# tangtang888/video-edge-ai-proxy

Hardware: AMD Instinct MI355X
Metric: decoded FPS (whole node) + p50 VideoLatestImage latency, 256×1080p RTSP (higher is better)
Workload: dtype uint8 (BGR24 frames; bf16-capable consumer path)

## Files before the change

csrc/vep/gpu_avc.hip:

```cpp
#define VEP_KERNEL_SOURCE 1
#include "avc_recon.h"
#include "gpu.h"

namespace vep::gpu {

using avc::MbRec;
using avc::kDenseCoefs;

namespace {

constexpr int kIntraWaves = kAvcDbkWgRows;
constexpr int kIntraXgWords = 8;
constexpr int kIntraLine = 32;
constexpr int kIntraLineCols = 240;
constexpr u32 kSpinLimit = 1u << 24;

__device__ inline const MbRec& rec(const AvcDesc& d, int mb) {
  return static_cast<const MbRec*>(d.mbs)[mb];
}


__device__ inline void wave_sync() {
  __builtin_amdgcn_fence(__ATOMIC_RELEASE, "wavefront");
  __builtin_amdgcn_wave_barrier();
// ... 435 lines not shown
        avc::intra16x16_const_from_sums(m.i16_mode, B, A, st, sl, H, V, P(15, -1), P(-1, 15));
    auto T = [&](int xx) { return P(xx, -1); };
    auto Lf = [&](int yy) { return P(-1, yy); };
    u8 out[4];
    for (int k = 0; k < 4; ++k) {
      const int p = lane + 64 * k, px = p & 15, py = p >> 4;
      out[k] = u8(avc::clip1(avc::intra16x16_pred_g(T, Lf, pk, m.i16_mode, px, py) + L.res[p]));
    }
    wave_sync();
    for (int k = 0; k < 4; ++k) {
      const int p = lane + 64 * k;
      L.tile[((p >> 4) + 1) * kTp + (p & 15) + 1] = out[k];
    }
  } else if (m.kind == avc::kI8x8) {
    const int px = lane & 7, py = lane >> 3;
    for (int q = 0; q < 4; ++q) {
      const int bx = q & 1, by = q >> 1;
      const bool top = by > 0 || B, left = bx > 0 || A;
      const bool tl = (bx > 0 && by > 0) || (bx == 0 && by == 0 ? D : bx == 0 ? A : B);
      const bool tr = by == 0 ? (bx == 0 ? B : C) : (bx == 0);
      const u8* nb = &L.tile[(by * 8) * kTp + bx * 8];
      const int mode = avc::i4_mode(m, q);
      const int rs = L.res[(by * 8 + py) * 16 + bx * 8 + px];
      const u32 pw = tap8_lut[mode * 64 + lane];
      if (lane < 25) {
        const u32 fw = avc::intra8x8_filter_tap(top, left, tl, lane);
        auto off = [&](u32 u) -> int { return u > 16 ? int(u - 16) * kTp : (u >= 9 && !tr) ? 8 : int(u); };
        const int s0 = nb[off(fw & 31)], s1 = nb[off((fw >> 5) & 31)], s2 = nb[off((fw >> 10) & 31)];
        const int fv = avc::eval_tap8(fw, s0, s1, s2);
        L.pf[lane] = u8((fw & avc::kTap8Const) ? 128 : fv);
      }
      wave_sync();
      int v;
      if (mode == 2) {
        int sv = lane < 8 ? (top ? int(L.pf[1 + lane]) : 0) : lane < 16 ? (left ? int(L.pf[9 + lane]) : 0) : 0;
        for (int o = 8; o > 0; o >>= 1) sv += __shfl_xor(sv, o);
        sv = __shfl(sv, 0);
        v = top && left ? (sv + 8) >> 4 : (top || left) ? (sv + 4) >> 3 : 128;
      } else {
        v = avc::eval_tap8(pw, L.pf[pw & 31], L.pf[(pw >> 5) & 31], L.pf[(pw >> 10) & 31]);
      }
      L.tile[(by * 8 + py + 1) * kTp + bx * 8 + px + 1] = u8(avc::clip1(v + rs));
      wave_sync();
    }
  } else {
    for (int k = 0; k < 4; ++k) {
      const int p = lane + 64 * k, px = p & 15, py = p >> 4, bx = px >> 2, byy = py >> 2;
      const int r = byy * 4 + bx;
      const u32 tw = tap_lut[avc::i4_mode(m, r) * 16 + (py & 3) * 4 + (px & 3)];
      u32 word;
      if (tw & avc::kTapDc) {
        word = 1u << 31 | u32(byy > 0 || B) << 21 | u32(bx > 0 || A) << 22;
      } else {
        const bool tr = byy == 0 ? (bx < 3 ? B : C)
                                 : (bx < 3 && avc::raster_to_blk((byy - 1) * 4 + bx + 1) < avc::raster_to_blk(r));
        auto rel = [&](u32 n) -> u32 {
          return n == 0 ? 0u : n <= 8 ? 1u + ((n - 1 >= 4 && !tr) ? 3u : n - 1) : (n - 8) * u32(kTp);
        };
        word = rel(tw & 15) | rel((tw >> 4) & 15) << 7 | rel((tw >> 8) & 15) << 14 | ((tw >> 12) & 1023u) << 21;
      }
      L.taps[p] = word;
    }
    wave_sync();
    const int g = lane >> 4, i = (lane >> 2) & 3, j = lane & 3;
    auto slot = [&](int st) -> int {
      const int y_lo = st > 3 ? (st - 2) / 2 : 0, y_hi = st / 2 < 3 ? st / 2 : 3;
      const int yy = y_lo + g;
      return g < 2 && yy <= y_hi ? (yy * 4 + i) * 16 + (st - 2 * yy) * 4 + j : -1;
    };
    u32 tws[10];
    int rss[10];
#pragma unroll
    for (int st = 0; st < 10; ++st) {
      const int p = slot(st);
      tws[st] = p >= 0 ? L.taps[p] : 0u;
      rss[st] = p >= 0 ? L.res[p] : 0;
    }
#pragma unroll
    for (int st = 0; st < 10; ++st) {
      const int p = slot(st);
      if (p >= 0) {
        const int yy = p >> 6, bx = (p & 15) >> 2;
        const u32 tw = tws[st];
        const u8* nb = &L.tile[(yy * 4) * kTp + bx * 4];
        int v;
        if (tw >> 31) {
          int st4 = 0, sl4 = 0;
          for (int q = 0; q < 4; ++q) {
            st4 += nb[1 + q];
            sl4 += nb[(q + 1) * kTp];
          }
          const bool ht = (tw >> 21) & 1, hl = (tw >> 22) & 1;
          v = ht && hl ? (st4 + sl4 + 4) >> 3 : hl ? (sl4 + 2) >> 2 : ht ? (st4 + 2) >> 2 : 128;
        } else {
          const int n0 = nb[tw & 127], n1 = nb[(tw >> 7) & 127], n2 = nb[(tw >> 14) & 127];
          v = (int((tw >> 21) & 3) * n0 + int((tw >> 23) & 3) * n1 + int((tw >> 25) & 3) * n2 +
               int((tw >> 27) & 3)) >> int((tw >> 29) & 3);
        }
        v += rss[st];
        L.tile[(yy * 4 + i + 1) * kTp + bx * 4 + j + 1] = u8(avc::clip1(v));
      }
      wave_sync();
    }
  }
  const u64 t_luma = d.prof ? clock64() : 0;
  {
    u8 out[2];
    for (int k = 0; k < 2; ++k) {
      const int p = lane + 64 * k, c = p >> 6, q = p & 63, px = q & 7, py = q >> 3;
      const u8* t = L.ctile[c];
      auto T = [&](int xx) { return int(t[xx + 1]); };
      auto Lf = [&](int yy) { return int(t[(yy + 1) * kCp]); };
      const avc::PredConst pk =
          m.chroma_mode == 3 ? avc::chroma_plane_const_g(T, Lf) : avc::PredConst{0, 0, 0, 0};
      out[k] = u8(avc::clip1(avc::chroma_pred_g(T, Lf, B, A, pk, m.chroma_mode, px, py) + L.res[256 + p]));
    }
    wave_sync();
    for (int k = 0; k < 2; ++k) {
      const int p = lane + 64 * k, c = p >> 6, q = p & 63;
      L.ctile[c][((q >> 3) + 1) * kCp + (q & 7) + 1] = out[k];
    }
  }
  wave_sync();
  const u64 t_chroma = d.prof ? clock64() : 0;
  {
    const int ry = lane >> 2, rx = (lane & 3) * 4;
    const u8* src = &L.tile[(ry + 1) * kTp + rx + 1];
    const u32 w = u32(src[0]) | u32(src[1]) << 8 | u32(src[2]) << 16 | u32(src[3]) << 24;
    gst4(Y + size_t(y0 + ry) * pitch + x0 + rx, w);
    if (xi_out && lane >= 60) xg_put(xi_out + size_t(x) * kAvcXgWords + (lane - 60), w, 1u);
    if (line_out && lane >= 60) *(VEP_LDS u32*)(line_out + x * kIntraLine + (lane - 60) * 4) = w;
    if (lane < 32) {
      const int cyr = lane >> 2, cxb = (lane & 3) * 2;
      const u8* c0 = &L.ctile[0][(cyr + 1) * kCp + cxb + 1];
      const u8* c1 = &L.ctile[1][(cyr + 1) * kCp + cxb + 1];
      const u32 cw = u32(c0[0]) | u32(c1[0]) << 8 | u32(c0[1]) << 16 | u32(c1[1]) << 24;
      gst4(UV + size_t(row * 8 + cyr) * pitch + (x * 8 + cxb) * 2, cw);
      if (xi_out && lane >= 28) xg_put(xi_out + size_t(x) * kAvcXgWords + 4 + (lane - 28), cw, 1u);
      if (line_out && lane >= 28) *(VEP_LDS u32*)(line_out + x * kIntraLine + 16 + (lane - 28) * 4) = cw;
    }
    if (lane < 16) L.carry[lane] = L.tile[(lane + 1) * kTp + 16];
    if (lane < 16) L.ccarry[lane >> 3][lane & 7] = L.ctile[lane >> 3][((lane & 7) + 1) * kCp + 8];
  }
  wave_sync();
  if (d.prof) {
    __builtin_amdgcn_fence(__ATOMIC_RELEASE, "workgroup");
    const u64 t_end = clock64();
    acc[1] += t_loaded - t_start - waited;
    acc[2] += t_luma - t_res;
    acc[6] += t_res - t_loaded;
    acc[3] += t_chroma - t_luma;
    acc[4] += t_end - t_chroma;
    acc[5] += 1;
  }
}

__global__ __launch_bounds__(64 * kIntraWaves) void avc_intra_kernel(const AvcDesc* __restrict__ descs,
                                                                      int n, int groups) {
  const int b = int(blockIdx.x), j = b >> 3;
  const int pic = (j / groups) * 8 + (b & 7), grp = j % groups;
  if (pic >= n) return;
  const AvcDesc d = descs[pic];
  const int W = d.wmbs, H = d.hmbs, g0 = grp * kIntraWaves;
  if (g0 >= H || d.bd > 8 || d.cf == 2) return;
  __shared__ Sync sync;
  __shared__ IntraWave lds[kIntraWaves];
  __shared__ u32 tap_lut[9 * 16];
  __shared__ u32 tap8_lut[9 * 64];
  __shared__ u8 lines[kIntraWaves - 1][kIntraLineCols * kIntraLine];
  for (int t = int(threadIdx.x); t < 9 * 16; t += int(blockDim.x)) {
    const int mode = t >> 4, y = (t >> 2) & 3, x = t & 3;
    tap_lut[t] = mode == 2 ? avc::kTapDc : avc::pack_taps(avc::intra4x4_taps(mode, x, y));
  }
  for (int t = int(threadIdx.x); t < 9 * 64; t += int(blockDim.x))
    tap8_lut[t] = avc::intra8x8_pred_tap(t >> 6, t & 7, (t >> 3) & 7);
  sync_init(sync, kIntraWaves);
  const int wave = int(threadIdx.x) >> 6, lane = int(threadIdx.x) & 63;
  IntraWave& L = lds[wave];
  const MbRec* recs = static_cast<const MbRec*>(d.mbs);
  const int row = g0 + wave;
  const bool xin = grp > 0 && wave == 0;
  u64* xi_in = xin ? d.xg + size_t(grp - 1) * W * kAvcXgWords : nullptr;
  u64* xi_out = wave == kIntraWaves - 1 && row + 1 < H ? d.xg + size_t(grp) * W * kAvcXgWords : nullptr;
  const bool use_lines = W <= kIntraLineCols;
  const u8* line_in = use_lines && wave > 0 ? lines[wave - 1] : nullptr;
  u8* line_out = use_lines && wave + 1 < kIntraWaves ? lines[wave] : nullptr;
  u64 acc[7] = {0, 0, 0, 0, 0, 0, 0};
  if (row < H) {
    int prev = -2;
    for (int base = 0; base < W; base += 64) {
      const int x = base + lane;
      bool intra = false;
      if (x < W) {
        constexpr int kWords = int(sizeof(MbRec) / sizeof(uint2));
        const uint2* src = reinterpret_cast<const uint2*>(&recs[row * W + x]);
        uint2* dst = reinterpret_cast<uint2*>(&L.rec[lane]);
        uint2 q[kWords];
        for (int k = 0; k < kWords; ++k) q[k] = gld8(src + k);
        for (int k = 0; k < kWords; ++k) dst[k] = q[k];
        intra = avc::is_wave_intra(u8(q[0].x & 0xff));
      }
      if (row > 0)
        for (int q = lane; q < 66; q += 64) {
          const int ax = base - 1 + q;
          u8 v = 0;
          if (ax >= 0 && ax < W) {
            v = avc::is_wave_intra(u8(gld1(&recs[(row - 1) * W + ax].kind)));
          }
          L.up[q] = v;
        }
      const u64 mask = __ballot(intra);
      wave_sync();
      for (u64 bits = mask; bits; bits &= bits - 1) {
        const int xx = base + __ffsll(static_cast<unsigned long long>(bits)) - 1;
        const u64 t0 = d.prof ? clock64() : 0;
        publish_row(sync, wave, u32(xx));
        intra_mb(d, L, L.rec[xx - base], xx, row, prev == xx - 1, lane, tap_lut, tap8_lut, t0, acc, sync, wave,
                 wave > 0 ? u32(xx + 2 < W ? xx + 2 : W) : 0u, xi_in, row > 0 ? &L.up[1] - base : nullptr,
                 line_in, line_out, xi_out);
        prev = xx;
      }
    }
    publish_row(sync, wave, u32(W));
  }
  if (d.prof && lane == 0) {
    for (int k = 0; k < 6; ++k) atomicAdd(&d.prof[k], acc[k]);
    atomicAdd(&d.prof[11], acc[6]);
  }
}


__global__ __launch_bounds__(256) void avc_bs_kernel(const AvcDesc* __restrict__ descs, int n,
                                                      int total) {
  const int g = int(blockIdx.x) * 256 + int(threadIdx.x);
  if (g >= total) return;
  int lo = 0, hi = n - 1;
  while (lo < hi) {
    const int mid = (lo + hi + 1) >> 1;
    if (descs[mid].mb_begin <= g) lo = mid;
    else hi = mid - 1;
  }
  const AvcDesc d = descs[lo];
  const int mb = g - d.mb_begin, W = d.wmbs, x = mb % W, row = mb / W;
  if (row % kAvcDbkWgRows == kAvcDbkWgRows - 1 && row + 1 < d.hmbs) {
    uint4* z = reinterpret_cast<uint4*>(
        d.xg + (size_t(row / kAvcDbkWgRows) * W + x) * kAvcXgWords);
    for (int k = 0; k < kAvcXgWords / 2; ++k) z[k] = make_uint4(0, 0, 0, 0);
  }
  const MbRec q = rec(d, mb);
  AvcDbkInfo info{};
  if (!(q.dbk & 1)) {
    const MbRec lm = rec(d, x > 0 ? mb - 1 : mb);
    const MbRec tm = rec(d, row > 0 ? mb - W : mb);
    const bool left = x > 0 && !((q.dbk & 2) && lm.slice != q.slice);
    const bool top = row > 0 && !((q.dbk & 2) && tm.slice != q.slice);
    const i16* mq = avc::is_intra(q.kind) ? nullptr : d.mvs + size_t(q.mv);
    const i16* ml = avc::is_intra(lm.kind) ? nullptr : d.mvs + size_t(lm.mv);
    const i16* mt = avc::is_intra(tm.kind) ? nullptr : d.mvs + size_t(tm.mv);
    const bool t8 = (q.flags & avc::kMbT8x8) != 0;
    const avc::BsSide sq = avc::bs_side(q), sl = avc::bs_side(lm), st = avc::bs_side(tm);
    u64 bsw[2] = {0, 0};
    for (int dir = 0; dir < 2; ++dir)
      for (int e = 0; e < 4; ++e) {
        if (e == 0 && !(dir == 0 ? left : top)) continue;
        if ((e & 1) && t8 && !(d.cf == 2 && dir == 1)) continue;
        const avc::BsSide p = e > 0 ? sq : (dir == 0 ? sl : st);
        const i16* mp = e > 0 ? mq : (dir == 0 ? ml : mt);
        for (int sg = 0; sg < 4; ++sg) {
          const int bq = dir == 0 ? sg * 4 + e : e * 4 + sg;
          const int bp = e > 0 ? (dir == 0 ? bq - 1 : bq - 4) : (dir == 0 ? bq + 3 : bq + 12);
          const int bs = avc::boundary_strength(p, bp, mp, sq, bq, mq, e == 0, d.field != 0, dir == 0);
          const u64 v = u64(bs) << (4 * (e * 4 + sg));
          if (dir == 0) bsw[0] |= v;
          else bsw[1] |= v;
        }
      }
    info.bs[0] = u32(bsw[0]);
    info.bs[1] = u32(bsw[0] >> 32);
    info.bs[2] = u32(bsw[1]);
    info.bs[3] = u32(bsw[1] >> 32);
    info.any = (bsw[0] | bsw[1]) ? 1 : 0;
    const int qb = d.qp_bias, qcb = d.qpc_bias;
#pragma unroll
    for (int k = 0; k < 3; ++k) {
      const MbRec& pk = k == 0 ? lm : (k == 1 ? tm : q);
      const avc::EdgeParams ep[3] = {avc::edge_params(pk.qp - qb, q.qp - qb, q.alpha_off, q.beta_off),
                                     avc::edge_params(pk.qpc - qcb, q.qpc - qcb, q.alpha_off, q.beta_off),
                                     avc::edge_params(pk.qpc2 - qcb, q.qpc2 - qcb, q.alpha_off, q.beta_off)};
      for (int c = 0; c < 3; ++c) {
        info.alpha[c * 3 + k] = u8(ep[c].alpha);
        info.beta[c * 3 + k] = u8(ep[c].beta);
        for (int j = 0; j < 3; ++j) info.tc0[c * 3 + k][j] = u8(ep[c].tc0[j]);
      }
    }
  }
  static_cast<AvcDbkInfo*>(d.dbk)[mb] = info;
}


struct DbkWave {
  AvcDbkInfo info;
  u8 y[20 * 20];
  u8 c[2][10 * 12];
  u8 carry[16 * 4];
  u8 ccarry[2][8 * 2];
};

struct alignas(16) DbkXch {
  u8 y[4 * 16];
  u8 c[2 * 16];
};

constexpr int kDbkLag = 1;
constexpr int kDbkDepth = 8;
#ifndef VEP_DBK_WG_ROWS
#define VEP_DBK_WG_ROWS kAvcDbkWgRows
#endif
constexpr int kDbkRows = VEP_DBK_WG_ROWS;
constexpr int kDbkWaves = kDbkRows / 2;
constexpr u32 kXgFinal = 2u, kXgPartial = 1u;
static_assert(kDbkRows % 2 == 0 && kDbkDepth > kDbkLag && kDbkRows % kAvcDbkWgRows == 0 && kDbkRows <= 32,
              "deblock wavefront geometry");

struct DbkSync {
  u32 progress[kDbkRows];
  u32 abort;
};

__device__ inline void st4(u8* p, u32 v) { *reinterpret_cast<u32*>(p) = v; }
__device__ inline u32 ld4(const u8* p) { return *reinterpret_cast<const u32*>(p); }

__device__ inline void wait_row_lds(DbkSync& s, int r, u32 need, u32* err) {
  u32 spins = 0;
  while (__hip_atomic_load(&s.progress[r], __ATOMIC_RELAXED, __HIP_MEMORY_SCOPE_WORKGROUP) < need) {
    if (__hip_atomic_load(&s.abort, __ATOMIC_RELAXED, __HIP_MEMORY_SCOPE_WORKGROUP)) break;
    if (++spins > kSpinLimit) {
      __hip_atomic_store(&s.abort, 1u, __ATOMIC_RELAXED, __HIP_MEMORY_SCOPE_WORKGROUP);
      if ((threadIdx.x & 63) == 0) atomicOr(err, 2u);
      break;
    }
    __builtin_amdgcn_s_sleep(1);
  }
  __builtin_amdgcn_fence(__ATOMIC_ACQUIRE, "workgroup", "local");
}

__device__ inline int bs_of(const AvcDbkInfo& in, int dir, int e, int sg) {
  const int i = dir * 16 + e * 4 + sg;
  return int((in.bs[i >> 3] >> (4 * (i & 7))) & 15u);
}

__device__ inline bool filter_vals(int p0, int p1, int p2, int p3, int q0, int q1, int q2, int q3, int bs, int alpha,
                                   int beta, int tc0, bool chroma, int& np0, int& np1, int& np2, int& nq0, int& nq1,
                                   int& nq2) {
  if (!(avc::iabs(p0 - q0) < alpha && avc::iabs(p1 - p0) < beta && avc::iabs(q1 - q0) < beta)) return false;
  const int ap = avc::iabs(p2 - p0), aq = avc::iabs(q2 - q0);
  const bool lp = !chroma && ap < beta, lq = !chroma && aq < beta;
  np1 = p1;
  nq1 = q1;
  np2 = p2;
  nq2 = q2;
  if (bs < 4) {
    const int tc = chroma ? tc0 + 1 : tc0 + int(lp) + int(lq);
    const int dl = avc::clip3(-tc, tc, (((q0 - p0) << 2) + (p1 - q1) + 4) >> 3);
    np0 = avc::clip1(p0 + dl);
    nq0 = avc::clip1(q0 - dl);
    if (lp) np1 = p1 + avc::clip3(-tc0, tc0, (p2 + ((p0 + q0 + 1) >> 1) - (p1 << 1)) >> 1);
    if (lq) nq1 = q1 + avc::clip3(-tc0, tc0, (q2 + ((p0 + q0 + 1) >> 1) - (q1 << 1)) >> 1);
  } else {
    const bool strong = !chroma && avc::iabs(p0 - q0) < ((alpha >> 2) + 2);
    if (lp && strong) {
      np0 = (p2 + 2 * p1 + 2 * p0 + 2 * q0 + q1 + 4) >> 3;
      np1 = (p2 + p1 + p0 + q0 + 2) >> 2;
      np2 = (2 * p3 + 3 * p2 + p1 + p0 + q0 + 4) >> 3;
    } else {
      np0 = (2 * p1 + p0 + q1 + 2) >> 2;
    }
    if (lq && strong) {
      nq0 = (p1 + 2 * p0 + 2 * q0 + 2 * q1 + q2 + 4) >> 3;
      nq1 = (p0 + q0 + q1 + q2 + 2) >> 2;
      nq2 = (2 * q3 + 3 * q2 + q1 + q0 + p0 + 4) >> 3;
    } else {
      nq0 = (2 * q1 + q0 + p1 + 2) >> 2;
    }
  }
  return true;
}

__device__ inline void filter_vert_any(u8* q0p, int bs, int alpha, int beta, int tc0, bool chroma) {
  int p0, p1, p2, p3, q0, q1, q2, q3;
  u32 P = 0, Q = 0;
  if (!chroma) {
    const u32* w = reinterpret_cast<const u32*>(q0p - 4);
    P = w[0];
    Q = w[1];
    p3 = int(P & 255);
    p2 = int((P >> 8) & 255);
    p1 = int((P >> 16) & 255);
    p0 = int(P >> 24);
    q0 = int(Q & 255);
    q1 = int((Q >> 8) & 255);
    q2 = int((Q >> 16) & 255);
    q3 = int(Q >> 24);
  } else {
    const u16* h = reinterpret_cast<const u16*>(q0p - 2);
    P = h[0];
    Q = h[1];
    p1 = p2 = p3 = int(P & 255);
    p0 = int(P >> 8);
    q0 = int(Q & 255);
    q1 = q2 = q3 = int(Q >> 8);
  }
  int np0, np1, np2, nq0, nq1, nq2;
  if (!filter_vals(p0, p1, p2, p3, q0, q1, q2, q3, bs, alpha, beta, tc0, chroma, np0, np1, np2, nq0, nq1, nq2)) return;
  if (!chroma) {
    u32* w = reinterpret_cast<u32*>(q0p - 4);
    w[0] = (P & 255u) | u32(np2) << 8 | u32(np1) << 16 | u32(np0) << 24;
    w[1] = u32(nq0) | u32(nq1) << 8 | u32(nq2) << 16 | (Q & 0xFF000000u);
  } else {
    u16* h = reinterpret_cast<u16*>(q0p - 2);
    h[0] = u16((P & 255u) | u32(np0) << 8);
    h[1] = u16(u32(nq0) | (Q & 0xFF00u));
  }
}

__device__ inline void filter_line_any(u8* s, int step, int bs, int alpha, int beta, int tc0, bool chroma) {
  const int p0 = s[-step], p1 = s[-2 * step], q0 = s[0], q1 = s[step];
  const int p2 = s[-3 * step], p3 = s[-4 * step], q2 = s[2 * step], q3 = s[3 * step];
  if (!(avc::iabs(p0 - q0) < alpha && avc::iabs(p1 - p0) < beta && avc::iabs(q1 - q0) < beta)) return;
  const int ap = avc::iabs(p2 - p0), aq = avc::iabs(q2 - q0);
  const bool lp = !chroma && ap < beta, lq = !chroma && aq < beta;
  int np0, nq0, np1 = p1, nq1 = q1, np2 = p2, nq2 = q2;
  if (bs < 4) {
    const int tc = chroma ? tc0 + 1 : tc0 + int(lp) + int(lq);
    const int dl = avc::clip3(-tc, tc, (((q0 - p0) << 2) + (p1 - q1) + 4) >> 3);
    np0 = avc::clip1(p0 + dl);
    nq0 = avc::clip1(q0 - dl);
    if (lp) np1 = p1 + avc::clip3(-tc0, tc0, (p2 + ((p0 + q0 + 1) >> 1) - (p1 << 1)) >> 1);
    if (lq) nq1 = q1 + avc::clip3(-tc0, tc0, (q2 + ((p0 + q0 + 1) >> 1) - (q1 << 1)) >> 1);
  } else {
    const bool strong = !chroma && avc::iabs(p0 - q0) < ((alpha >> 2) + 2);
    if (lp && strong) {
      np0 = (p2 + 2 * p1 + 2 * p0 + 2 * q0 + q1 + 4) >> 3;
      np1 = (p2 + p1 + p0 + q0 + 2) >> 2;
      np2 = (2 * p3 + 3 * p2 + p1 + p0 + q0 + 4) >> 3;
    } else {
      np0 = (2 * p1 + p0 + q1 + 2) >> 2;
    }
    if (lq && strong) {
      nq0 = (p1 + 2 * p0 + 2 * q0 + 2 * q1 + q2 + 4) >> 3;
      nq1 = (p0 + q0 + q1 + q2 + 2) >> 2;
      nq2 = (2 * q3 + 3 * q2 + q1 + q0 + p0 + 4) >> 3;
    } else {
      nq0 = (2 * q1 + q0 + p1 + 2) >> 2;
    }
  }
  s[-step] = u8(np0);
  s[0] = u8(nq0);
  if (!chroma) {
    s[-2 * step] = u8(np1);
    s[step] = u8(nq1);
    s[-3 * step] = u8(np2);
    s[2 * step] = u8(nq2);
  }
}

__device__ inline void dbk_dir(DbkWave& L, bool any, int l, int dir, bool packed, bool sync_each) {
  const bool ch = l >= 16;
  const int c = (l - 16) >> 3, k = (l - 16) & 7;
  int bs[4], al[4], be[4], tc[4];
#pragma unroll
  for (int e = 0; e < 4; ++e) {
    bs[e] = any && (!ch || !(e & 1)) ? bs_of(L.info, dir, e, ch ? k >> 1 : l >> 2) : 0;
    const int pi = (e > 0 ? 2 : dir) + (ch ? 3 + 3 * c : 0);
    al[e] = L.info.alpha[pi];
    be[e] = L.info.beta[pi];
    tc[e] = L.info.tc0[pi][bs[e] > 0 && bs[e] < 4 ? bs[e] - 1 : 0];
  }
#pragma unroll
  for (int e = 0; e < 4; ++e) {
    if (bs[e] && dir == 0 && packed) {
      u8* q0p = !ch ? &L.y[(4 + l) * 20 + 4 + 4 * e] : &L.c[c][(2 + k) * 12 + 4 + 2 * e];
      filter_vert_any(q0p, bs[e], al[e], be[e], bs[e] < 4 ? tc[e] : 0, ch);
    } else if (bs[e]) {
      u8* sp;
      int step;
      if (!ch) {
        sp = dir == 0 ? &L.y[(4 + l) * 20 + 4 + 4 * e] : &L.y[(4 + 4 * e) * 20 + 4 + l];
        step = dir == 0 ? 1 : 20;
      } else {
        sp = dir == 0 ? &L.c[c][(2 + k) * 12 + 4 + 2 * e] : &L.c[c][(2 + 2 * e) * 12 + 4 + k];
        step = dir == 0 ? 1 : 12;
      }
      filter_line_any(sp, step, bs[e], al[e], be[e], bs[e] < 4 ? tc[e] : 0, ch);
    }
    if (sync_each) wave_sync();
  }
  if (!sync_each) wave_sync();
}

__device__ inline void dbk_dir_regs(DbkWave& L, bool any, int l, int dir) {
  const bool ch = l >= 16;
  const int c = (l - 16) >> 3, k = (l - 16) & 7;
  int bs[4], al[4], be[4], tc[4];
#pragma unroll
  for (int e = 0; e < 4; ++e) {
    const int ee = ch ? 2 * e : e;
    bs[e] = any && (!ch || e < 2) ? bs_of(L.info, dir, ee, ch ? k >> 1 : l >> 2) : 0;
    const int pi = (ee > 0 ? 2 : dir) + (ch ? 3 + 3 * c : 0);
    al[e] = L.info.alpha[pi];
    be[e] = L.info.beta[pi];
    tc[e] = L.info.tc0[pi][bs[e] > 0 && bs[e] < 4 ? bs[e] - 1 : 0];
  }
  u32 w[5] = {0, 0, 0, 0, 0};
  u8* row = !ch ? &L.y[(4 + l) * 20] : &L.c[c][(2 + k) * 12];
  u8* col = !ch ? &L.y[4 * 20 + 4 + l] : &L.c[c][2 * 12 + 4 + k];
  const int stride = ch ? 12 : 20, lo = ch ? 2 : 0, hi = ch ? 12 : 20, nw = ch ? 3 : 5;
  if (dir == 0) {
#pragma unroll
    for (int i = 0; i < 5; ++i)
      if (i < nw) w[i] = ld4(row + 4 * i);
  } else {
#pragma unroll
    for (int i = 0; i < 20; ++i)
      if (i >= lo && i < hi) w[i >> 2] |= u32(col[(i - 4) * stride]) << (8 * (i & 3));
  }
#pragma unroll
  for (int e = 0; e < 4; ++e) {
    if (!bs[e]) continue;
    const u32 P = w[e], Q = w[e + 1];
    int np0, np1, np2, nq0, nq1, nq2;
    if (!filter_vals(int(P >> 24), int((P >> 16) & 255), int((P >> 8) & 255), int(P & 255), int(Q & 255),
                     int((Q >> 8) & 255), int((Q >> 16) & 255), int(Q >> 24), bs[e], al[e], be[e],
                     bs[e] < 4 ? tc[e] : 0, ch, np0, np1, np2, nq0, nq1, nq2))
      continue;
    w[e] = (P & 255u) | u32(np2) << 8 | u32(np1) << 16 | u32(np0) << 24;
    w[e + 1] = u32(nq0) | u32(nq1) << 8 | u32(nq2) << 16 | (Q & 0xFF000000u);
  }
  if (dir == 0) {
#pragma unroll
    for (int i = 0; i < 5; ++i)
      if (i < nw) st4(row + 4 * i, w[i]);
  } else {
#pragma unroll
    for (int i = 1; i < 20; ++i)
      if (i >= lo && i < hi) col[(i - 4) * stride] = u8(w[i >> 2] >> (8 * (i & 3)));
  }
  wave_sync();
}

struct DbkRegs {
  u32 info, m0, m1, c;
};

__global__ __launch_bounds__(64 * kDbkWaves) void avc_deblock_kernel(const AvcDesc* __restrict__ descs,
                                                                      int n, int groups, int packed) {
  const int b = int(blockIdx.x), j = b >> 3;
  const int pic = (j / groups) * 8 + (b & 7), grp = j % groups;
  if (pic >= n) return;
  const AvcDesc d = descs[pic];
  const int W = d.wmbs, H = d.hmbs, pitch = W * 16;
  const int g0 = grp * kDbkRows;
  if (g0 >= H || d.bd > 8 || d.cf == 2) return;
  __shared__ DbkSync sync;
  __shared__ DbkWave lds[kDbkWaves][2];
  __shared__ DbkXch xring[kDbkRows - 1][kDbkDepth];
  if (threadIdx.x < kDbkRows) sync.progress[threadIdx.x] = 0;
  if (threadIdx.x == 0) sync.abort = 0;
  __syncthreads();
  const int wave = int(threadIdx.x) >> 6, lane = int(threadIdx.x) & 63;
  const int h = lane >> 5, l = lane & 31;
  DbkWave& L = lds[wave][h];
  u8* Y = d.y + d.slot_y * u64(d.target);
  u8* UV = d.uv + d.slot_uv * u64(d.target);
  const AvcDbkInfo* infos = static_cast<const AvcDbkInfo*>(d.dbk);
  auto xch = [&](int r, int x) -> DbkXch& { return xring[r - g0][x % kDbkDepth]; };
  auto load_mb = [&](int row, int x) {
    row = row < H ? row : H - 1;
    x = x < 0 ? 0 : (x < W ? x : W - 1);
    DbkRegs v;
    v.info = gld4(reinterpret_cast<const u32*>(&infos[size_t(row) * W + x]) + (l < 16 ? l : 0));
    const u8* ym = Y + size_t(row * 16 + (l >> 2)) * pitch + x * 16 + (l & 3) * 4;
    v.m0 = gld4(ym);
    v.m1 = gld4(ym + size_t(8) * pitch);
    v.c = gld4(UV + size_t(row * 8 + (l >> 2)) * pitch + x * 16 + (l & 3) * 4);
    return v;
  };
  const int r0 = g0 + 2 * wave, row = r0 + h, lrow = row - g0;
  const bool last = row == H - 1;
  const bool prod = row + 1 < H;
  const bool xout = prod && lrow == kDbkRows - 1;
  const bool xin = grp > 0 && wave == 0;
  const int xw = l >= 16 ? l - 16 : (l >= 8 ? 16 + (l - 8) : -1);
  const bool xneed = xin && h == 0 && xw >= 0;
  u64* xg_in = xin ? d.xg + size_t(grp - 1) * W * kAvcXgWords : nullptr;
  u64* xg_out = d.xg + size_t(grp) * W * kAvcXgWords;
  u64 gx = 0;
  if (xneed) gx = xg_get(xg_in + xw);
  u64 acc[5] = {0, 0, 0, 0, 0};
  DbkRegs cur = load_mb(row, -kDbkLag * h);
  for (int i = 0; r0 < H && i < W + kDbkLag; ++i) {
    const int x = i - h * kDbkLag;
    const bool act = row < H && x >= 0 && x < W;
    const u64 t0 = d.prof ? clock64() : 0;
    const DbkRegs nxt = load_mb(row, x + 1);
    {
      const int x1 = i - kDbkLag;
      if (r0 + 2 < H && wave + 1 < kDbkWaves && x1 < W && x1 - kDbkDepth + 2 > 0)
        wait_row_lds(sync, 2 * wave + 2, u32(x1 - kDbkDepth + 2), d.err);
    }
    const u64 t1 = d.prof ? clock64() : 0;
    const int x0 = x * 16, y0 = row * 16;
    if (act) {
      const u32 carry = ld4(&L.carry[(l & 15) * 4]);
      const int l7 = l & 7;
      const u8 cc0 = L.ccarry[0][l7 * 2], cc1 = L.ccarry[1][l7 * 2], cc2 = L.ccarry[0][l7 * 2 + 1],
               cc3 = L.ccarry[1][l7 * 2 + 1];
      if (l < 16) reinterpret_cast<u32*>(&L.info)[l] = cur.info;
      st4(&L.y[((l >> 2) + 4) * 20 + 4 + (l & 3) * 4], cur.m0);
      st4(&L.y[((l >> 2) + 12) * 20 + 4 + (l & 3) * 4], cur.m1);
      if (l < 16 && x > 0) st4(&L.y[(l + 4) * 20], carry);
      {
        const int cyr = l >> 2, cb = (l & 3) * 2;
        for (int q = 0; q < 2; ++q) {
          L.c[0][(cyr + 2) * 12 + 4 + cb + q] = u8(cur.c >> (16 * q));
          L.c[1][(cyr + 2) * 12 + 4 + cb + q] = u8(cur.c >> (16 * q + 8));
        }
      }
      if (l < 8 && x > 0) {
        L.c[0][(l + 2) * 12 + 2] = cc0;
        L.c[1][(l + 2) * 12 + 2] = cc1;
        L.c[0][(l + 2) * 12 + 3] = cc2;
        L.c[1][(l + 2) * 12 + 3] = cc3;
      }
    }
    wave_sync();
    const u64 t2 = d.prof ? clock64() : 0;
    const bool any = act && L.info.any;
    const bool wany = __ballot(any) != 0;
    if (wany) {
      if (packed & 4) dbk_dir_regs(L, any, l, 0);
      else dbk_dir(L, any, l, 0, (packed & 1) != 0, (packed & 2) != 0);
    }
    if (act && prod && x > 0) {
      u32 fw = 0;
      int fi = -1;
      if (l >= 24 && l < 28) {
        const int k = l - 24;
        fw = ld4(&L.y[(16 + k) * 20]);
        fi = k * 4 + 3;
      } else if (l >= 28 && l < 30) {
        const int k = l - 28, cr = 8 + k;
        fw = u32(L.c[0][cr * 12 + 2]) | u32(L.c[1][cr * 12 + 2]) << 8 | u32(L.c[0][cr * 12 + 3]) << 16 |
             u32(L.c[1][cr * 12 + 3]) << 24;
        fi = 16 + k * 4 + 3;
      }
      if (fi >= 0) {
        if (xout) xg_put(xg_out + size_t(x - 1) * kAvcXgWords + fi, fw, kXgFinal);
        else st4(fi < 16 ? &xch(row, x - 1).y[fi * 4] : &xch(row, x - 1).c[(fi - 16) * 4], fw);
      }
    }
    __builtin_amdgcn_fence(__ATOMIC_RELEASE, "workgroup", "local");
    if (l == 0 && act)
      __hip_atomic_store(&sync.progress[lrow], u32(x + 1), __ATOMIC_RELAXED, __HIP_MEMORY_SCOPE_WORKGROUP);
    const u64 t3 = d.prof ? clock64() : 0;
    if (xin && i < W) {
      u32 spins = 0;
      while (__ballot(xneed && u32(gx >> 32) != kXgFinal)) {
        if (__hip_atomic_load(&sync.abort, __ATOMIC_RELAXED, __HIP_MEMORY_SCOPE_WORKGROUP)) break;
        if (++spins > (kSpinLimit >> 4)) {
          __hip_atomic_store(&sync.abort, 1u, __ATOMIC_RELAXED, __HIP_MEMORY_SCOPE_WORKGROUP);
          if (lane == 0) atomicOr(d.err, 2u);
          break;
        }
        __builtin_amdgcn_s_sleep(1);
        if (xneed) gx = xg_get(xg_in + size_t(i) * kAvcXgWords + xw);
      }
    }
    const u32 gv = u32(gx);
    if (xneed && i + 1 < W) gx = xg_get(xg_in + size_t(i + 1) * kAvcXgWords + xw);
    if (wave > 0 && i < W) wait_row_lds(sync, 2 * wave - 1, u32(i + 2), d.err);
    wave_sync();
    const u64 t4 = d.prof ? clock64() : 0;
    const bool top_g = xin && h == 0;
    if (act && row > 0) {
      if (l >= 16) {
        const int k = l - 16;
        st4(&L.y[(k >> 2) * 20 + 4 + (k & 3) * 4], top_g ? gv : ld4(&xch(row - 1, x).y[k * 4]));
      } else if (l >= 8) {
        const int k = l - 8, tr = k >> 2, cb = (k & 3) * 2;
        const u32 v = top_g ? gv : ld4(&xch(row - 1, x).c[k * 4]);
        for (int q = 0; q < 2; ++q) {
          L.c[0][tr * 12 + 4 + cb + q] = u8(v >> (16 * q));
          L.c[1][tr * 12 + 4 + cb + q] = u8(v >> (16 * q + 8));
        }
      }
    }
    wave_sync();
    const u64 t5 = d.prof ? clock64() : 0;
    if (wany) {
      if (packed & 4) dbk_dir_regs(L, any, l, 1);
      else dbk_dir(L, any, l, 1, false, (packed & 2) != 0);
    }
    const u64 t6 = d.prof ? clock64() : 0;
    if (act) {
      const bool left = any && (L.info.bs[0] & 0xFFFFu) != 0;
      auto cbyte = [&](int c, int i) { return u32(L.c[c][i]); };
      auto cword = [&](int base) {
        return cbyte(0, base) | cbyte(1, base) << 8 | cbyte(0, base + 1) << 16 | cbyte(1, base + 1) << 24;
      };
      const int q4 = l >> 2, r4 = (l & 3) * 4, cb = (l & 3) * 2, k16 = (l - 16) & 15;
      const u32 w_top = ld4(&L.y[(q4 + 4) * 20 + 4 + r4]);
      const u32 w_bot = ld4(&L.y[(q4 + 12) * 20 + 4 + r4]);
      const u32 w_c = cword((q4 + 2) * 12 + 4 + cb);
      const u32 w_side = ld4(l < 16 ? &L.y[(l + 4) * 20]
                                    : &L.y[(k16 >> 2) * 20 + 4 + (k16 & 3) * 4]);
      const int l8 = l & 7, k8 = (l - 8) & 7;
      const u32 w_cside = l < 8 ? cword((l8 + 2) * 12 + 2)
                                : cword((k8 >> 2) * 12 + 4 + (k8 & 3) * 2);
      const int kx = (l - 16) & 7;
      const u32 w_x = l < 16 ? ld4(&L.y[(16 + q4) * 20 + 4 + r4])
                             : cword((8 + (kx >> 2)) * 12 + 4 + (kx & 3) * 2);
      const u32 w_carry = ld4(&L.y[((l & 15) + 4) * 20 + 16]);
      const int cc = ((l - 16) >> 3) & 1, ck = (l - 16) & 7;
      const u8 cr0 = L.c[cc][(ck + 2) * 12 + 10], cr1 = L.c[cc][(ck + 2) * 12 + 11];
      if (any) {
        u8* ym = Y + size_t(y0 + q4) * pitch + x0 + r4;
        gst4(ym, w_top);
        if (q4 < 4 || last) gst4(ym + size_t(8) * pitch, w_bot);
        if (q4 < 6 || last) gst4(UV + size_t(row * 8 + q4) * pitch + x0 + cb * 2, w_c);
      }
      if (l < 16) {
        if (left && (l < 12 || last)) gst4(Y + size_t(y0 + l) * pitch + x0 - 4, w_side);
      } else if (row > 0) {
        gst4(Y + size_t(y0 - 4 + (k16 >> 2)) * pitch + x0 + (k16 & 3) * 4, w_side);
      }
      if (l < 8) {
        if (left && (l < 6 || last)) gst4(UV + size_t(row * 8 + l) * pitch + x0 - 4, w_cside);
      } else if (l < 16 && row > 0) {
        gst4(UV + size_t(row * 8 - 2 + (k8 >> 2)) * pitch + x0 + (k8 & 3) * 4, w_cside);
      }
      if (prod && l < 24) {
        if (xout)
          xg_put(xg_out + size_t(x) * kAvcXgWords + l, w_x, (l & 3) == 3 && x + 1 < W ? kXgPartial : kXgFinal);
        else
          st4(l < 16 ? &xch(row, x).y[l * 4] : &xch(row, x).c[(l - 16) * 4], w_x);
      }
      if (l < 16) {
        st4(&L.carry[l * 4], w_carry);
      } else {
        L.ccarry[cc][ck * 2] = cr0;
        L.ccarry[cc][ck * 2 + 1] = cr1;
      }
    }
    if (x == W - 1) {
      __builtin_amdgcn_fence(__ATOMIC_RELEASE, "workgroup", "local");
      if (l == 0 && act)
        __hip_atomic_store(&sync.progress[lrow], u32(W + 1), __ATOMIC_RELAXED, __HIP_MEMORY_SCOPE_WORKGROUP);
    }
    wave_sync();
    cur = nxt;
    if (d.prof) {
      const u64 t7 = clock64();
      acc[0] += (t1 - t0) + (t4 - t3);
      acc[1] += (t2 - t1) + (t5 - t4);
      acc[2] += (t3 - t2) + (t6 - t5);
      acc[3] += t7 - t6;
      acc[4] += u64(__popcll(__ballot(act) & 0x100000001ull));
    }
  }
  if (d.prof && lane == 0)
    for (int k = 0; k < 5; ++k) atomicAdd(&d.prof[6 + k], acc[k]);
}

__global__ __launch_bounds__(256) void weave_kernel(const WeaveDesc* __restrict__ descs) {
  const WeaveDesc d = descs[blockIdx.y];
  const u8* __restrict__ y = d.y;
  const u8* __restrict__ uv = d.uv;
  u8* __restrict__ y8 = d.y8;
  u8* __restrict__ uv8 = d.uv8;
  const int pitch = d.pitch, h = d.height;
  const int per_row = pitch / 16;
  const size_t g = size_t(blockIdx.x) * 256 + threadIdx.x, total = size_t(per_row) * size_t(h + h / 2);
  if (g >= total) return;
  const int row = int(g / size_t(per_row)), col = int(g % size_t(per_row)) * 16;
  const bool luma = row < h;
  const int r = luma ? row : row - h, fh = luma ? h / 2 : h / 4;
  const u8* src = (luma ? y : uv) + (size_t(r & 1) * size_t(fh) + size_t(r >> 1)) * size_t(pitch) + size_t(col);
  u8* dst = (luma ? y8 : uv8) + size_t(r) * size_t(pitch) + size_t(col);
  *reinterpret_cast<uint4*>(dst) = *reinterpret_cast<const uint4*>(src);
}

}

void launch_weave(const WeaveDesc* d_descs, int n, int max_pitch, int max_height, hipStream_t s) {
  if (n <= 0 || max_pitch <= 0 || max_height <= 0) return;
  const size_t lanes = size_t(max_pitch / 16) * size_t(max_height + max_height / 2);
  hipLaunchKernelGGL(weave_kernel, dim3(unsigned((lanes + 255) / 256), unsigned(n)), dim3(256), 0, s, d_descs);
  VEP_HIP(hipGetLastError());
}

void launch_avc_inter(const AvcDesc* d_descs, int n, int total_mbs, hipStream_t s) {
  if (n <= 0 || total_mbs <= 0) return;
  hipLaunchKernelGGL(avc_inter_kernel, dim3(unsigned((total_mbs + 3) / 4)), dim3(256), 0, s, d_descs, n,
                     total_mbs);
  VEP_HIP(hipGetLastError());
}

void launch_avc_intra(const AvcDesc* d_descs, int n, int max_hmbs, hipStream_t s) {
  if (n <= 0 || max_hmbs <= 0) return;
  const int groups = avc_dbk_groups(max_hmbs);
  const unsigned blocks = unsigned((n + 7) / 8) * unsigned(groups) * 8u;
  hipLaunchKernelGGL(avc_intra_kernel, dim3(blocks), dim3(64 * kIntraWaves), 0, s, d_descs, n, groups);
  VEP_HIP(hipGetLastError());
}

void launch_avc_bs(const AvcDesc* d_descs, int n, int total_mbs, hipStream_t s) {
  if (n <= 0 || total_mbs <= 0) return;
  hipLaunchKernelGGL(avc_bs_kernel, dim3(unsigned((total_mbs + 255) / 256)), dim3(256), 0, s, d_descs,
                     n, total_mbs);
  VEP_HIP(hipGetLastError());
}

void launch_avc_deblock(const AvcDesc* d_descs, int n, int max_hmbs, hipStream_t s, int packed) {
  if (n <= 0 || max_hmbs <= 0) return;
  const int groups = (max_hmbs + kDbkRows - 1) / kDbkRows;
  const unsigned blocks = unsigned((n + 7) / 8) * unsigned(groups) * 8u;
  hipLaunchKernelGGL(avc_deblock_kernel, dim3(blocks), dim3(64 * kDbkWaves), 0, s, d_descs, n, groups, packed);
  VEP_HIP(hipGetLastError());
}

}
```

Before: 8496.

## Use DPP quad transposes and word-wide LDS access in register deblock path

Reworks the register-based H.264 deblock path. Vertical-edge columns are now loaded as 4-byte words and transposed inside lane quads with DPP and perm, replacing byte-by-byte strided LDS access. Boundary-strength words are preloaded from global memory, and chroma planes are split with byte permutes instead of per-byte stores. The separate carry buffers are dropped so carried columns are written directly into the working tile. The aim is fewer LDS instructions and bank conflicts, at the cost of extra cross-lane shuffles, an extra 16-byte global load per macroblock, and subtle correctness risk in the lane-index remapping.

```diff
diff --git a/csrc/vep/gpu_avc.hip b/csrc/vep/gpu_avc.hip
--- a/csrc/vep/gpu_avc.hip
+++ b/csrc/vep/gpu_avc.hip
@@ -761,8 +761,6 @@
   AvcDbkInfo info;
   u8 y[20 * 20];
   u8 c[2][10 * 12];
-  u8 carry[16 * 4];
-  u8 ccarry[2][8 * 2];
 };
 
 struct alignas(16) DbkXch {
@@ -957,58 +955,81 @@
   if (!sync_each) wave_sync();
 }
 
-__device__ inline void dbk_dir_regs(DbkWave& L, bool any, int l, int dir) {
+struct DbkPar {
+  int bs[4], al[4], be[4], tc[4];
+};
+
+__device__ inline void dbk_params(const DbkWave& L, u32 blo, u32 bhi, bool any, int l, int dir, DbkPar& p) {
   const bool ch = l >= 16;
   const int c = (l - 16) >> 3, k = (l - 16) & 7;
-  int bs[4], al[4], be[4], tc[4];
+  const int sg = ch ? k >> 1 : l >> 2;
 #pragma unroll
   for (int e = 0; e < 4; ++e) {
     const int ee = ch ? 2 * e : e;
-    bs[e] = any && (!ch || e < 2) ? bs_of(L.info, dir, ee, ch ? k >> 1 : l >> 2) : 0;
+    const u32 word = (ee & 2) ? bhi : blo;
+    p.bs[e] = any && (!ch || e < 2) ? int((word >> (4 * ((ee & 1) * 4 + sg))) & 15u) : 0;
     const int pi = (ee > 0 ? 2 : dir) + (ch ? 3 + 3 * c : 0);
-    al[e] = L.info.alpha[pi];
-    be[e] = L.info.beta[pi];
-    tc[e] = L.info.tc0[pi][bs[e] > 0 && bs[e] < 4 ? bs[e] - 1 : 0];
-  }
+    p.al[e] = L.info.alpha[pi];
+    p.be[e] = L.info.beta[pi];
+    p.tc[e] = L.info.tc0[pi][p.bs[e] > 0 && p.bs[e] < 4 ? p.bs[e] - 1 : 0];
+  }
+}
+
+__device__ inline u32 quad_xor1(u32 v) { return u32(__builtin_amdgcn_update_dpp(0, int(v), 0xB1, 0xF, 0xF, false)); }
+__device__ inline u32 quad_xor2(u32 v) { return u32(__builtin_amdgcn_update_dpp(0, int(v), 0x4E, 0xF, 0xF, false)); }
+__device__ inline u32 row_shr8(u32 v) { return u32(__builtin_amdgcn_update_dpp(0, int(v), 0x118, 0xF, 0xF, false)); }
+
+__device__ inline u32 quad_transpose(u32 r, u32 s1, u32 s2) {
+  const u32 u = __builtin_amdgcn_perm(quad_xor1(r), r, s1);
+  return __builtin_amdgcn_perm(quad_xor2(u), u, s2);
+}
+__device__ inline u32 quad_sel1(int lane) { return (lane & 1) ? 0x03070105u : 0x06020400u; }
+__device__ inline u32 quad_sel2(int lane) { return (lane & 2) ? 0x03020706u : 0x05040100u; }
+
+__device__ inline u32 dbk_dir_regs(DbkWave& L, const DbkPar& p, int l, int dir) {
+  const bool ch = l >= 16;
+  const int c = (l - 16) >> 3, k = (l - 16) & 7;
   u32 w[5] = {0, 0, 0, 0, 0};
-  u8* row = !ch ? &L.y[(4 + l) * 20] : &L.c[c][(2 + k) * 12];
-  u8* col = !ch ? &L.y[4 * 20 + 4 + l] : &L.c[c][2 * 12 + 4 + k];
-  const int stride = ch ? 12 : 20, lo = ch ? 2 : 0, hi = ch ? 12 : 20, nw = ch ? 3 : 5;
-  if (dir == 0) {
-#pragma unroll
-    for (int i = 0; i < 5; ++i)
-      if (i < nw) w[i] = ld4(row + 4 * i);
-  } else {
-#pragma unroll
-    for (int i = 0; i < 20; ++i)
-      if (i >= lo && i < hi) w[i >> 2] |= u32(col[(i - 4) * stride]) << (8 * (i & 3));
+  const int stride = ch ? 12 : 20, nw = ch ? 3 : 5;
+  const int j = l & 3, g = ch ? k >> 2 : l >> 2;
+  u8* line = dir == 0 ? (!ch ? &L.y[(4 + l) * 20] : &L.c[c][(2 + k) * 12])
+                      : (!ch ? &L.y[j * 20 + 4 + 4 * g] : &L.c[c][0] + (j - 2) * 12 + 4 + 4 * g);
+  const int step = dir == 0 ? 4 : 4 * stride;
+  const u32 s1 = quad_sel1(l), s2 = quad_sel2(l);
+#pragma unroll
+  for (int i = 0; i < 5; ++i)
+    if (i < nw) w[i] = ld4(line + step * i);
+  if (dir == 1) {
+#pragma unroll
+    for (int i = 0; i < 5; ++i) w[i] = quad_transpose(w[i], s1, s2);
   }
 #pragma unroll
   for (int e = 0; e < 4; ++e) {
-    if (!bs[e]) continue;
+    if (!p.bs[e]) continue;
     const u32 P = w[e], Q = w[e + 1];
     int np0, np1, np2, nq0, nq1, nq2;
     if (!filter_vals(int(P >> 24), int((P >> 16) & 255), int((P >> 8) & 255), int(P & 255), int(Q & 255),
-                     int((Q >> 8) & 255), int((Q >> 16) & 255), int(Q >> 24), bs[e], al[e], be[e],
-                     bs[e] < 4 ? tc[e] : 0, ch, np0, np1, np2, nq0, nq1, nq2))
+                     int((Q >> 8) & 255), int((Q >> 16) & 255), int(Q >> 24), p.bs[e], p.al[e], p.be[e],
+                     p.bs[e] < 4 ? p.tc[e] : 0, ch, np0, np1, np2, nq0, nq1, nq2))
       continue;
     w[e] = (P & 255u) | u32(np2) << 8 | u32(np1) << 16 | u32(np0) << 24;
     w[e + 1] = u32(nq0) | u32(nq1) << 8 | u32(nq2) << 16 | (Q & 0xFF000000u);
   }
-  if (dir == 0) {
-#pragma unroll
-    for (int i = 0; i < 5; ++i)
-      if (i < nw) st4(row + 4 * i, w[i]);
-  } else {
-#pragma unroll
-    for (int i = 1; i < 20; ++i)
-      if (i >= lo && i < hi) col[(i - 4) * stride] = u8(w[i >> 2] >> (8 * (i & 3)));
-  }
+  const u32 first = w[0];
+  if (dir == 1) {
+#pragma unroll
+    for (int i = 0; i < 5; ++i) w[i] = quad_transpose(w[i], s1, s2);
+  }
+#pragma unroll
+  for (int i = 0; i < 5; ++i)
+    if (i < nw && !(dir == 1 && ch && i == 0 && j < 2)) st4(line + step * i, w[i]);
   wave_sync();
+  return first;
 }
 
 struct DbkRegs {
   u32 info, m0, m1, c;
+  u32 b0, b1, b2, b3;
 };
 
 __global__ __launch_bounds__(64 * kDbkWaves) void avc_deblock_kernel(const AvcDesc* __restrict__ descs,
@@ -1038,6 +1059,8 @@
     x = x < 0 ? 0 : (x < W ? x : W - 1);
     DbkRegs v;
     v.info = gld4(reinterpret_cast<const u32*>(&infos[size_t(row) * W + x]) + (l < 16 ? l : 0));
+    const uint4 bs = gld16(&infos[size_t(row) * W + x]);
+    v.b0 = bs.x, v.b1 = bs.y, v.b2 = bs.z, v.b3 = bs.w;
     const u8* ym = Y + size_t(row * 16 + (l >> 2)) * pitch + x * 16 + (l & 3) * 4;
     v.m0 = gld4(ym);
     v.m1 = gld4(ym + size_t(8) * pitch);
@@ -1069,49 +1092,41 @@
     }
     const u64 t1 = d.prof ? clock64() : 0;
     const int x0 = x * 16, y0 = row * 16;
+    const u32 sel_pl = (l & 1) ? 0x03010705u : 0x06040200u;
+    const u32 cpl = __builtin_amdgcn_perm(quad_xor1(cur.c), cur.c, sel_pl);
     if (act) {
-      const u32 carry = ld4(&L.carry[(l & 15) * 4]);
-      const int l7 = l & 7;
-      const u8 cc0 = L.ccarry[0][l7 * 2], cc1 = L.ccarry[1][l7 * 2], cc2 = L.ccarry[0][l7 * 2 + 1],
-               cc3 = L.ccarry[1][l7 * 2 + 1];
       if (l < 16) reinterpret_cast<u32*>(&L.info)[l] = cur.info;
       st4(&L.y[((l >> 2) + 4) * 20 + 4 + (l & 3) * 4], cur.m0);
       st4(&L.y[((l >> 2) + 12) * 20 + 4 + (l & 3) * 4], cur.m1);
-      if (l < 16 && x > 0) st4(&L.y[(l + 4) * 20], carry);
-      {
-        const int cyr = l >> 2, cb = (l & 3) * 2;
-        for (int q = 0; q < 2; ++q) {
-          L.c[0][(cyr + 2) * 12 + 4 + cb + q] = u8(cur.c >> (16 * q));
-          L.c[1][(cyr + 2) * 12 + 4 + cb + q] = u8(cur.c >> (16 * q + 8));
-        }
-      }
-      if (l < 8 && x > 0) {
-        L.c[0][(l + 2) * 12 + 2] = cc0;
-        L.c[1][(l + 2) * 12 + 2] = cc1;
-        L.c[0][(l + 2) * 12 + 3] = cc2;
-        L.c[1][(l + 2) * 12 + 3] = cc3;
-      }
+      st4(&L.c[l & 1][((l >> 2) + 2) * 12 + 4 + ((l & 3) >> 1) * 4], cpl);
     }
     wave_sync();
     const u64 t2 = d.prof ? clock64() : 0;
-    const bool any = act && L.info.any;
+    const bool any = act && (cur.b0 | cur.b1 | cur.b2 | cur.b3) != 0;
     const bool wany = __ballot(any) != 0;
-    if (wany) {
-      if (packed & 4) dbk_dir_regs(L, any, l, 0);
-      else dbk_dir(L, any, l, 0, (packed & 1) != 0, (packed & 2) != 0);
-    }
+    const bool regs = (packed & 4) != 0;
+    DbkPar p0, p1;
+    if (wany && regs) {
+      dbk_params(L, cur.b0, cur.b1, any, l, 0, p0);
+      dbk_params(L, cur.b2, cur.b3, any, l, 1, p1);
+    }
+    u32 w0;
+    if (wany && regs) {
+      w0 = dbk_dir_regs(L, p0, l, 0);
+    } else {
+      if (wany) dbk_dir(L, any, l, 0, (packed & 1) != 0, (packed & 2) != 0);
+      w0 = ld4(l < 16 ? &L.y[(4 + l) * 20] : &L.c[(l - 16) >> 3][(2 + ((l - 16) & 7)) * 12]);
+    }
+    const u32 w0cb = row_shr8(w0);
     if (act && prod && x > 0) {
       u32 fw = 0;
       int fi = -1;
-      if (l >= 24 && l < 28) {
-        const int k = l - 24;
-        fw = ld4(&L.y[(16 + k) * 20]);
-        fi = k * 4 + 3;
-      } else if (l >= 28 && l < 30) {
-        const int k = l - 28, cr = 8 + k;
-        fw = u32(L.c[0][cr * 12 + 2]) | u32(L.c[1][cr * 12 + 2]) << 8 | u32(L.c[0][cr * 12 + 3]) << 16 |
-             u32(L.c[1][cr * 12 + 3]) << 24;
-        fi = 16 + k * 4 + 3;
+      if (l >= 12 && l < 16) {
+        fw = w0;
+        fi = (l - 12) * 4 + 3;
+      } else if (l >= 30) {
+        fw = __builtin_amdgcn_perm(w0cb, w0, 0x03070206u);
+        fi = 16 + (l - 30) * 4 + 3;
       }
       if (fi >= 0) {
         if (xout) xg_put(xg_out + size_t(x - 1) * kAvcXgWords + fi, fw, kXgFinal);
@@ -1141,47 +1156,48 @@
     wave_sync();
     const u64 t4 = d.prof ? clock64() : 0;
     const bool top_g = xin && h == 0;
-    if (act && row > 0) {
-      if (l >= 16) {
-        const int k = l - 16;
-        st4(&L.y[(k >> 2) * 20 + 4 + (k & 3) * 4], top_g ? gv : ld4(&xch(row - 1, x).y[k * 4]));
-      } else if (l >= 8) {
-        const int k = l - 8, tr = k >> 2, cb = (k & 3) * 2;
-        const u32 v = top_g ? gv : ld4(&xch(row - 1, x).c[k * 4]);
-        for (int q = 0; q < 2; ++q) {
-          L.c[0][tr * 12 + 4 + cb + q] = u8(v >> (16 * q));
-          L.c[1][tr * 12 + 4 + cb + q] = u8(v >> (16 * q + 8));
+    {
+      const DbkXch& tx = xring[lrow > 0 ? lrow - 1 : 0][(act ? x : 0) % kDbkDepth];
+      const u32 tv = top_g ? gv : ld4(l >= 16 ? &tx.y[(l - 16) * 4] : &tx.c[(l & 7) * 4]);
+      const u32 tpl = __builtin_amdgcn_perm(quad_xor1(tv), tv, sel_pl);
+      if (act && row > 0) {
+        if (l >= 16) {
+          const int k = l - 16;
+          st4(&L.y[(k >> 2) * 20 + 4 + (k & 3) * 4], tv);
+        } else if (l >= 8) {
+          const int k = l - 8;
+          st4(&L.c[l & 1][(k >> 2) * 12 + 4 + ((k & 3) >> 1) * 4], tpl);
         }
       }
     }
     wave_sync();
     const u64 t5 = d.prof ? clock64() : 0;
     if (wany) {
-      if (packed & 4) dbk_dir_regs(L, any, l, 1);
+      if (regs) dbk_dir_regs(L, p1, l, 1);
       else dbk_dir(L, any, l, 1, false, (packed & 2) != 0);
     }
     const u64 t6 = d.prof ? clock64() : 0;
     if (act) {
-      const bool left = any && (L.info.bs[0] & 0xFFFFu) != 0;
-      auto cbyte = [&](int c, int i) { return u32(L.c[c][i]); };
-      auto cword = [&](int base) {
-        return cbyte(0, base) | cbyte(1, base) << 8 | cbyte(0, base + 1) << 16 | cbyte(1, base + 1) << 24;
+      const bool left = any && (cur.b0 & 0xFFFFu) != 0;
+      auto cword = [&](int r, int cb) {
+        const int o = r * 12 + 4 + (cb & ~3);
+        return __builtin_amdgcn_perm(ld4(&L.c[0][o]), ld4(&L.c[1][o]), (cb & 2) ? 0x03070206u : 0x01050004u);
       };
       const int q4 = l >> 2, r4 = (l & 3) * 4, cb = (l & 3) * 2, k16 = (l - 16) & 15;
       const u32 w_top = ld4(&L.y[(q4 + 4) * 20 + 4 + r4]);
       const u32 w_bot = ld4(&L.y[(q4 + 12) * 20 + 4 + r4]);
-      const u32 w_c = cword((q4 + 2) * 12 + 4 + cb);
+      const u32 w_c = cword(q4 + 2, cb);
       const u32 w_side = ld4(l < 16 ? &L.y[(l + 4) * 20]
                                     : &L.y[(k16 >> 2) * 20 + 4 + (k16 & 3) * 4]);
       const int l8 = l & 7, k8 = (l - 8) & 7;
-      const u32 w_cside = l < 8 ? cword((l8 + 2) * 12 + 2)
-                                : cword((k8 >> 2) * 12 + 4 + (k8 & 3) * 2);
+      const u32 w_cside = l < 8 ? cword(l8 + 2, -2)
+                                : cword(k8 >> 2, (k8 & 3) * 2);
       const int kx = (l - 16) & 7;
       const u32 w_x = l < 16 ? ld4(&L.y[(16 + q4) * 20 + 4 + r4])
-                             : cword((8 + (kx >> 2)) * 12 + 4 + (kx & 3) * 2);
+                             : cword(8 + (kx >> 2), (kx & 3) * 2);
       const u32 w_carry = ld4(&L.y[((l & 15) + 4) * 20 + 16]);
       const int cc = ((l - 16) >> 3) & 1, ck = (l - 16) & 7;
-      const u8 cr0 = L.c[cc][(ck + 2) * 12 + 10], cr1 = L.c[cc][(ck + 2) * 12 + 11];
+      const u16 w_ccarry = *reinterpret_cast<const u16*>(&L.c[cc][(ck + 2) * 12 + 10]);
       if (any) {
         u8* ym = Y + size_t(y0 + q4) * pitch + x0 + r4;
         gst4(ym, w_top);
@@ -1204,12 +1220,8 @@
         else
           st4(l < 16 ? &xch(row, x).y[l * 4] : &xch(row, x).c[(l - 16) * 4], w_x);
       }
-      if (l < 16) {
-        st4(&L.carry[l * 4], w_carry);
-      } else {
-        L.ccarry[cc][ck * 2] = cr0;
-        L.ccarry[cc][ck * 2 + 1] = cr1;
-      }
+      if (l < 16) st4(&L.y[(l + 4) * 20], w_carry);
+      else *reinterpret_cast<u16*>(&L.c[cc][(ck + 2) * 12 + 2]) = w_ccarry;
     }
     if (x == W - 1) {
       __builtin_amdgcn_fence(__ATOMIC_RELEASE, "workgroup", "local");
```

Result: slower. 8388 (-1.3%).
